# LucaHermes/ddrl

Hardware: AMD Instinct MI355X
Metric: env-steps/sec at 4096 envs × 4 leg agents; PPO update ms/minibatch (higher is better)
Workload: dtype fp32

## Files before the change

### ddrl_amd/csrc/common.h

```cpp
#pragma once
#include <hip/hip_runtime.h>
#include <stdint.h>

typedef float floatx4 __attribute__((ext_vector_type(4)));
typedef unsigned v4u __attribute__((ext_vector_type(4)));

#define DDRL_H 64
#ifndef DDRL_MB
#define DDRL_MB 128
#endif
#define DDRL_LOG2PI 1.8378770664093453

#ifndef DDRL_LDS_PAD
#define DDRL_LDS_PAD 1
#endif
constexpr bool kLdsPad = DDRL_LDS_PAD != 0;
__host__ __device__ constexpr int lds_rs(bool pad) { return pad ? 80 : 64; }
__host__ __device__ constexpr int lds_blk(bool pad) { return 16 * lds_rs(pad); }
__host__ __device__ constexpr int lds_img(int rows, bool pad) { return rows * lds_rs(pad); }
#define DDRL_LBLK lds_blk(kLdsPad)
#define DDRL_LIMG(rows) lds_img(rows, kLdsPad)
template <bool PAD = kLdsPad>
__device__ __forceinline__ int swz(int row) { return PAD ? (row & 0xB) : (((row >> 1) & 7) << 1); }
template <bool PAD = kLdsPad>
// ... 303 lines not shown
    }
}

template <int RT, bool PAD = kLdsPad>
__device__ __forceinline__ void layer2_bwd_rt(const NetLds& W, const floatx4 (*dz2)[4], floatx4 (*dh1)[4]) {
  constexpr int BLK = lds_blk(PAD);
#pragma unroll
  for (int t = 0; t < RT; ++t)
#pragma unroll
    for (int fb = 0; fb < 4; ++fb) dh1[t][fb] = splat4(0.f);
  const int wb[4] = {wbase<PAD>(0), wbase<PAD>(1), wbase<PAD>(2), wbase<PAD>(3)};
  auto ld = [&](int k, float* a) {
    const float* wp = W.w2 + wb[k & 3] + 16 * (k >> 2);
#pragma unroll
    for (int fb = 0; fb < 4; ++fb) a[fb] = wp[BLK * fb];
  };
  float wr[3][4];
  ld(0, wr[0]);
  ld(1, wr[1]);
#pragma unroll
  for (int k = 0; k < 16; ++k) {
    if (k + 2 < 16) ld(k + 2, wr[(k + 2) % 3]);
#pragma unroll
    for (int fb = 0; fb < 4; ++fb)
#pragma unroll
      for (int t = 0; t < RT; ++t) dh1[t][fb] = mfma4(wr[k % 3][fb], dz2[t][k >> 2][k & 3], dh1[t][fb]);
    __builtin_amdgcn_sched_barrier(0);
  }
}
__device__ __forceinline__ void layer2_bwd(const NetLds& W, const floatx4 dz2[4], floatx4 dh1[4]) {
  layer2_bwd_rt<1>(W, reinterpret_cast<const floatx4 (*)[4]>(dz2), reinterpret_cast<floatx4 (*)[4]>(dh1));
}

__device__ __forceinline__ void store_act(float* buf, int tile, const floatx4 v[4]) {
#pragma unroll
  for (int r = 0; r < 4; ++r) {
    float* p = buf + wbase(r) + DDRL_LBLK * tile;
#pragma unroll
    for (int fb = 0; fb < 4; ++fb) p[16 * fb] = v[fb][r];
  }
}

#define FM_LD 136
template <int LD = FM_LD>
__device__ __forceinline__ void store_act_fm(float* buf, int tile, const floatx4 v[4]) {
  const int lane = threadIdx.x & 63, c = lane & 15, q = lane >> 4;
  float* p = buf + (4 * q) * LD + 16 * tile + c;
#pragma unroll
  for (int fb = 0; fb < 4; ++fb)
#pragma unroll
    for (int r = 0; r < 4; ++r) p[(16 * fb + r) * LD] = v[fb][r];
}

template <int NROWS, int NT_, int LD = NROWS + 8, bool AHEAD = true>
__device__ __forceinline__ void dw_tiles_fm(const float* A, const float* B, const int* fa, int fo, floatx4* out) {
  const int lane = threadIdx.x & 63, c = lane & 15, q = lane >> 4;
#pragma unroll
  for (int i = 0; i < NT_; ++i) out[i] = splat4(0.f);
  const float* bp = B + (16 * fo + c) * LD + 4 * q;
  const float* ap[NT_];
#pragma unroll
  for (int i = 0; i < NT_; ++i) ap[i] = A + (16 * fa[i] + c) * LD + 4 * q;
  constexpr int NU = NROWS / 16;
  floatx4 bv[2], av[2][NT_];
  if constexpr (!AHEAD) {
    bv[0] = *reinterpret_cast<const floatx4*>(bp);
#pragma unroll
    for (int i = 0; i < NT_; ++i) av[0][i] = *reinterpret_cast<const floatx4*>(ap[i]);
#pragma unroll
    for (int u = 0; u < NU; ++u) {
      if (u + 1 < NU) {
        bv[(u + 1) & 1] = *reinterpret_cast<const floatx4*>(bp + 16 * (u + 1));
#pragma unroll
        for (int i = 0; i < NT_; ++i) av[(u + 1) & 1][i] = *reinterpret_cast<const floatx4*>(ap[i] + 16 * (u + 1));
      }
#pragma unroll
      for (int i = 0; i < NT_; ++i)
#pragma unroll
        for (int v = 0; v < 4; ++v) out[i] = mfma4(av[u & 1][i][v], bv[u & 1][v], out[i]);
      __builtin_amdgcn_sched_barrier(0);
    }
  } else {
    auto ld = [&](int u, int j) {
      if (j < NT_) av[u & 1][j] = *reinterpret_cast<const floatx4*>(ap[j] + 16 * u);
      else bv[u & 1] = *reinterpret_cast<const floatx4*>(bp + 16 * u);
    };
    constexpr int NL = NT_ + 1, PER = (NL + 2) / 3;
#pragma unroll
    for (int j = 0; j < NL; ++j) ld(0, j);
#pragma unroll
    for (int u = 0; u < NU; ++u) {
      __builtin_amdgcn_sched_barrier(0);
#pragma unroll
      for (int v = 0; v < 4; ++v) {
        if (u + 1 < NU && v < 3) {
#pragma unroll
          for (int j = v * PER; j < (v + 1) * PER && j < NL; ++j) ld(u + 1, j);
          __builtin_amdgcn_sched_barrier(0);
        }
#pragma unroll
        for (int i = 0; i < NT_; ++i) out[i] = mfma4(av[u & 1][i][v], bv[u & 1][v], out[i]);
        __builtin_amdgcn_sched_barrier(0);
      }
    }
  }
}

template <int NROWS>
__device__ __forceinline__ floatx4 dw_tile(const float* A, const float* B, int fa, int fo) {
  floatx4 acc = splat4(0.f);
  const int rb[4] = {rbase(0), rbase(1), rbase(2), rbase(3)};
  const float* ap = A + 16 * fa;
  const float* bp = B + 16 * fo;
#pragma unroll 2
  for (int u = 0; u < NROWS / 16; ++u) {
#pragma unroll
    for (int v = 0; v < 4; ++v) acc = mfma4(ap[rb[v] + DDRL_LBLK * u], bp[rb[v] + DDRL_LBLK * u], acc);
  }
  return acc;
}

template <int NROWS>
__device__ __forceinline__ void dw_tile2(const float* A, const float* B, int fa0, int fo0, int fa1, int fo1,
                                         floatx4& t0, floatx4& t1) {
  floatx4 a0 = splat4(0.f), a1 = splat4(0.f);
  const int rb[4] = {rbase(0), rbase(1), rbase(2), rbase(3)};
  const float *ap0 = A + 16 * fa0, *bp0 = B + 16 * fo0, *ap1 = A + 16 * fa1, *bp1 = B + 16 * fo1;
#pragma unroll 2
  for (int u = 0; u < NROWS / 16; ++u) {
#pragma unroll
    for (int v = 0; v < 4; ++v) {
      const int o = rb[v] + DDRL_LBLK * u;
      a0 = mfma4(ap0[o], bp0[o], a0);
      a1 = mfma4(ap1[o], bp1[o], a1);
    }
  }
  t0 = a0;
  t1 = a1;
}

template <int O, int NROWS>
__device__ __forceinline__ floatx4 dw_tile_head(const float* A, const float* D, int fa) {
  const int lane = threadIdx.x & 63, c = lane & 15, q = lane >> 4;
  floatx4 acc = splat4(0.f);
  const int rb[4] = {rbase(0), rbase(1), rbase(2), rbase(3)};
  const float* ap = A + 16 * fa;
  const bool cv = c < O;
  const float* dp = D + q * O + (cv ? c : 0);
#pragma unroll 2
  for (int u = 0; u < NROWS / 16; ++u) {
#pragma unroll
// ... 8 lines not shown
```

### ddrl_amd/csrc/ppo_ffn_impl.h

```cpp
#pragma once
#include <atomic>
#include "common.h"
#include "kernels.h"
#include "ffn.h"
#include "ppo_loss.h"

#ifndef DDRL_FFN_AT
#define DDRL_FFN_AT 0
#endif

#ifndef DDRL_FFN_KSP
#define DDRL_FFN_KSP 0
#endif
#ifndef DDRL_FFN_GROUP
#define DDRL_FFN_GROUP 0
#endif
#if DDRL_FFN_GROUP && (DDRL_FFN_KSP != 2 || DDRL_FFN_AT || DDRL_MB != 128 || defined(DDRL_XCHG_ATOMIC) || \
                       defined(DDRL_BOUNDS) || defined(DDRL_STAMPS))
#error "the group unit builds the production fused row-split kernel only (KSP = 2, 128 rows, default protocol)"
#endif
#if DDRL_MB == 256
#if DDRL_FFN_KSP != 2 || DDRL_FFN_AT == 2
#error "the DDRL_MB = 256 units build the fused row-split kernels only (DDRL_FFN_KSP = 2, no peer mode)"
#endif
#if DDRL_FFN_AT
#define DDRL_FFN_LAUNCH launch_update_ffn_mb256_atomic
#else
#define DDRL_FFN_LAUNCH launch_update_ffn_mb256
#endif
#elif DDRL_MB != 128
#error "DDRL_MB must be 128 or 256"
#elif DDRL_FFN_KSP == 1
#define DDRL_FFN_LAUNCH launch_update_ffn_k1
#elif DDRL_FFN_AT == 2
#define DDRL_FFN_LAUNCH launch_update_ffn_peer
#elif DDRL_FFN_AT
#define DDRL_FFN_LAUNCH launch_update_ffn_atomic
#else
#define DDRL_FFN_LAUNCH launch_update_ffn
#endif
#if DDRL_FFN_AT || defined(DDRL_XCHG_ATOMIC)
#define DDRL_XCHG_IS_ATOMIC 1
#else
#define DDRL_XCHG_IS_ATOMIC 0
#endif
#define DDRL_XCHG_LXSYS (DDRL_FFN_AT == 2)
#define DDRL_LX_ON (!DDRL_XCHG_IS_ATOMIC || DDRL_XCHG_LXSYS)
#ifndef DDRL_HEAD_PF
#define DDRL_HEAD_PF 4
#endif
constexpr int kHeadPfMaxO = (DDRL_FFN_KSP == 2 && !DDRL_FFN_AT) ? DDRL_HEAD_PF : 0;

namespace {

// ... 98 lines not shown
  for (int i = threadIdx.x; i < 64 * OB; i += blockDim.x) W.wo[i] = th[bo.wo + i];
  for (int i = threadIdx.x; i < OB; i += blockDim.x) W.bo[i] = th[bo.bo + i];
}
template <int OB, int NT, bool PAD>
__device__ __forceinline__ void stage_branch_batched(const float* __restrict__ th, int d, const BranchOff& bo,
                                                     float* lds, NetLds& W, int ncup) {
  static_assert((48 * 64) % NT == 0 && (64 * 64) % NT == 0, "staging split");
  constexpr int N1 = 48 * 64 / NT, N2 = 64 * 64 / NT, NS = (64 * OB + OB + 128 + NT - 1) / NT;
  W.w1 = lds; W.w2 = W.w1 + lds_img(48, PAD); W.b1 = W.w2 + lds_img(64, PAD); W.b2 = W.b1 + 64;
  W.wo = W.b2 + 64; W.bo = W.wo + 64 * OB; W.cup = W.bo + OB;
  const int t = threadIdx.x;
  float a1[N1], a2[N2], as[NS];
#pragma unroll
  for (int k = 0; k < N1; ++k) {
    const int i = t + NT * k;
    a1[k] = (i >> 6) < d ? th[bo.w1 + i] : 0.f;
  }
#pragma unroll
  for (int k = 0; k < N2; ++k) a2[k] = th[bo.w2 + t + NT * k];
#pragma unroll
  for (int k = 0; k < NS; ++k) {
    int e = t + NT * k;
    float x = 0.f;
    if (e < 64 * OB) x = th[bo.wo + e];
    else if ((e -= 64 * OB) < OB) x = th[bo.bo + e];
    else if ((e -= OB) < 64) x = th[bo.b1 + e];
    else if ((e -= 64) < 64) x = th[bo.b2 + e];
    as[k] = x;
  }
  float ac = t < ncup ? th[bo.cup + t] : 0.f;
#pragma unroll
  for (int k = 0; k < N1; ++k) {
    const int i = t + NT * k;
    W.w1[sidx<PAD>(i >> 6, i & 63)] = a1[k];
  }
#pragma unroll
  for (int k = 0; k < N2; ++k) {
    const int i = t + NT * k;
    W.w2[sidx<PAD>(i >> 6, i & 63)] = a2[k];
  }
#pragma unroll
  for (int k = 0; k < NS; ++k) {
    int e = t + NT * k;
    if (e < 64 * OB) W.wo[e] = as[k];
    else if ((e -= 64 * OB) < OB) W.bo[e] = as[k];
    else if ((e -= OB) < 64) W.b1[e] = as[k];
    else if ((e -= 64) < 64) W.b2[e] = as[k];
  }
  if (t < ncup) W.cup[t] = ac;
}
__host__ __device__ constexpr int branch_lds_floats(bool pad) { return lds_img(48, pad) + lds_img(64, pad) + 128 + 64 * 16 + 16; }
__host__ __device__ constexpr bool update_pad(int A, int ksp) { return kLdsPad && !(A == 8 && DDRL_MB / ksp >= 128); }
__host__ __device__ constexpr bool update_hmf(int ksp) { return ksp == 2 && DDRL_MB / ksp == 64; }

template <int OB>
__device__ __forceinline__ void small_param(int e, const BranchOff& bo, const NetLds& W, int& pidx, float*& lp) {
  if (e < 64 * OB) { pidx = bo.wo + e; lp = W.wo + e; return; }
  e -= 64 * OB;
  if (e < OB) { pidx = bo.bo + e; lp = W.bo + e; return; }
  e -= OB;
  if (e < 64) { pidx = bo.b1 + e; lp = W.b1 + e; return; }
  e -= 64;
  if (e < 64) { pidx = bo.b2 + e; lp = W.b2 + e; return; }
  e -= 64;
  pidx = bo.cup + e; lp = W.cup + e;
}


template <int A, int RT>
struct RowData {
  float x[RT][12];
  float act[RT][A];
  float ol[RT][2 * A];
  float s0[RT], s1[RT];
  int cid[RT];
};

template <int NW, int ROWS>
struct RowGather {
  static constexpr int MI = (ROWS * 20 + 64 * (NW - 1) - 1) / (64 * (NW - 1));
  const float* src[MI];
};
template <int NW, int ROWS>
__device__ __forceinline__ void rows_prepare(RowGather<NW, ROWS>& G, const float* rec, int stride, int cpr, int cpr_l,
                                             float inv_cpr_l, const int* idxb, int R) {
  constexpr int MI = RowGather<NW, ROWS>::MI;
  const int lane = threadIdx.x & 63, w = __builtin_amdgcn_readfirstlane(threadIdx.x >> 6);
#pragma unroll
  for (int it = 0; it < MI; ++it) G.src[it] = rec;
  if (w == NW - 1) return;
  const int nchunk = ROWS * cpr_l;
  int idx[MI], kk[MI];
#pragma unroll
  for (int it = 0; it < MI; ++it) {
    const int g = 64 * w + 64 * (NW - 1) * it + lane;
    int row = (int)(((float)g + 0.5f) * inv_cpr_l);
    kk[it] = min(g - row * cpr_l, cpr - 1);
    idx[it] = 0;
    if (g < nchunk) {
      if (!BCHK(row >= 0 && row < ROWS && kk[it] >= 0, 0)) row = 0;
      idx[it] = idxb[row];
    }
  }
#pragma unroll
  for (int it = 0; it < MI; ++it) {
    int i = idx[it];
// ... 316 lines not shown
  for (;;) {
#pragma unroll
    for (int j = 0; j < NQ; ++j)
      asm volatile("buffer_load_dwordx4 %0, %1, %2, %3 offen sc1" : "=v"(g[j]) : "v"(voff), "s"(rs), "s"(j * 4096));
    __builtin_amdgcn_sched_barrier(0);
    if (first) after_first();
    __builtin_amdgcn_sched_barrier(0);
    asm volatile("s_waitcnt vmcnt(0)" ::: "memory");
#pragma unroll
    for (int j = 0; j < NQ; ++j) asm volatile("" : "+v"(g[j]));
    unsigned bad = 0;
#pragma unroll
    for (int j = 0; j < NQ; ++j) bad |= (g[j][0] ^ bit) | (g[j][1] ^ bit) | (g[j][2] ^ bit) | (g[j][3] ^ bit);
#ifdef DDRL_STAMPS
    if (first && __builtin_amdgcn_ballot_w64((bad & 1u) != 0)) ++stale;
#endif
    first = false;
    if ((bad & 1u) == 0) break;
    if (xchg_abandon(t0, err)) {
#pragma unroll
      for (int j = 0; j < NQ; ++j) g[j] = v4u{0u, 0u, 0u, 0u};
      lost = true;
      break;
    }
    __builtin_amdgcn_s_sleep(1);
  }
  (void)stale;
#pragma unroll
  for (int j = 0; j < NQ; ++j)
#pragma unroll
    for (int k = 0; k < 4; ++k) out[4 * j + k] = __uint_as_float(g[j][k]);
  return lost;
}
#endif
#endif

template <int O>
__device__ __forceinline__ void head_bwd_mfma(const NetLds& W, const float* dout, floatx4 dh[4]) {
  static_assert(O % 4 == 0, "policy head: 2A outputs");
  const int lane = threadIdx.x & 63, c = lane & 15, q = lane >> 4;
  float b[O / 4];
#pragma unroll
  for (int kk = 0; kk < O / 4; ++kk)
    b[kk] = q == 0 ? dout[4 * kk] : q == 1 ? dout[4 * kk + 1] : q == 2 ? dout[4 * kk + 2] : dout[4 * kk + 3];
#pragma unroll
  for (int fb = 0; fb < 4; ++fb) {
    floatx4 acc = splat4(0.f);
#pragma unroll
    for (int kk = 0; kk < O / 4; ++kk) acc = mfma4(W.wo[(16 * fb + c) * O + 4 * kk + q], b[kk], acc);
    dh[fb] = acc;
  }
}

template <int NROWS, int NT_, int LD = NROWS + 8>
__device__ __forceinline__ void dw_tiles_fm_head(const float* A, const float* B, const int* fa, int fo, floatx4* out,
                                                 const float* AH, const float* BH, int fah, floatx4& outh) {
  const int lane = threadIdx.x & 63, c = lane & 15, q = lane >> 4;
#pragma unroll
  for (int i = 0; i < NT_; ++i) out[i] = splat4(0.f);
  outh = splat4(0.f);
  const float* bp = B + (16 * fo + c) * LD + 4 * q;
  const float* bph = BH + c * LD + 4 * q;
  const float* aph = AH + (16 * fah + c) * LD + 4 * q;
  const float* ap[NT_];
#pragma unroll
  for (int i = 0; i < NT_; ++i) ap[i] = A + (16 * fa[i] + c) * LD + 4 * q;
  constexpr int NU = NROWS / 16;
  floatx4 bv[2], av[2][NT_], bhv[2], ahv[2];
  auto ld = [&](int u, int j) {
    if (j < NT_) av[u & 1][j] = *reinterpret_cast<const floatx4*>(ap[j] + 16 * u);
    else if (j == NT_) bv[u & 1] = *reinterpret_cast<const floatx4*>(bp + 16 * u);
    else if (j == NT_ + 1) ahv[u & 1] = *reinterpret_cast<const floatx4*>(aph + 16 * u);
    else bhv[u & 1] = *reinterpret_cast<const floatx4*>(bph + 16 * u);
  };
  constexpr int NL = NT_ + 3, PER = (NL + 2) / 3;
#pragma unroll
  for (int j = 0; j < NL; ++j) ld(0, j);
#pragma unroll
  for (int u = 0; u < NU; ++u) {
    __builtin_amdgcn_sched_barrier(0);
#pragma unroll
    for (int v = 0; v < 4; ++v) {
      if (u + 1 < NU && v < 3) {
#pragma unroll
        for (int j = v * PER; j < (v + 1) * PER && j < NL; ++j) ld(u + 1, j);
        __builtin_amdgcn_sched_barrier(0);
      }
#pragma unroll
      for (int i = 0; i < NT_; ++i) out[i] = mfma4(av[u & 1][i][v], bv[u & 1][v], out[i]);
      outh = mfma4(ahv[u & 1][v], bhv[u & 1][v], outh);
      __builtin_amdgcn_sched_barrier(0);
    }
  }
}

template <int A, int KS1, int OB, bool POL, int NW, int KSP, bool CUP, bool LSBX>
__device__ __forceinline__ void update_loop(const UpdateArgs& U, const UpdateBatch& ub, float* lds, int p, int kq) {
  constexpr int ROWS = DDRL_MB / KSP;
  constexpr int NT = Geo<NW, ROWS>::NT, RT = Geo<NW, ROWS>::RT, NS1 = Geo<NW, ROWS>::NS1, NS2 = Geo<NW, ROWS>::NS2;
  constexpr bool PAD = update_pad(A, KSP);
  constexpr bool DWF = KSP != 1;
  const int wkq = ub.own_kq < 0 ? 0 : ub.own_kq;
  const UpdateHyper& H = ub.h;
  const int d = U.d;
  const FfnOffsets of = ffn_offsets(d, A);
  const BranchOff bo = branch_off(of, POL);
  const int nf1 = (d + 15) >> 4;
  constexpr int NSB0 = 64 * OB + OB + 128;
  constexpr int NCUP = CUP ? ncup_slots(OB, POL) : 0;
  constexpr int NSB = NSB0 + NCUP;
  constexpr bool cup = NCUP > 0;
  constexpr int nsb = NSB;
  constexpr int NSLOT = (NSB + NT - 1) / NT;
  constexpr int NSTAT = POL ? 3 : 5;
  constexpr int NTS = NS1 + NS2;
  constexpr int NP0 = (NSLOT + 2) / 2;
  constexpr int NP = NP0 + 2 * NTS;
  static_assert(KSP == 1 || (NT == 256 && NP == gx_pairs(OB, NW) && NP <= GX_MAX_PAIRS), "exchange pairs");
  constexpr bool LX = LSBX && KSP == 2 && DDRL_LX_ON;
  constexpr int NQ0 = (NSLOT + 1 + 3) / 4;
  constexpr int NQ = NQ0 + NTS;
  static_assert(!LX || NQ <= GX_MAX_PAIRS, "exchange quads");

  NetLds W;
  constexpr int LD = ROWS + 8;
  float* bufA = lds + branch_lds_floats(PAD);
  float* bufB = bufA + 64 * LD;
  float* Pb = bufB + 64 * LD;
  float* red = Pb + NW * NSB;
  int* idxb = reinterpret_cast<int*>(red + 128);
  static_assert(ROWS <= 128 && ROWS <= NT, "idxb holds 128 rows, one staging slot per thread");
  constexpr bool HMF = POL && update_hmf(KSP);
  float* bufH = red + 256;
  float* bufD = bufH + 64 * LD;
  float* stg = red + 256 + (HMF ? 80 * LD : 0);
  const int stride = U.lay.stride, cpr = stride >> 2, cpr_l = stg_chunks(stride, A);
  const float inv_cpr_l = 1.f / (float)cpr_l;

  const int tid = threadIdx.x, lane = tid & 63, c = lane & 15, q = lane >> 4,
            w = __builtin_amdgcn_readfirstlane(tid >> 6);
  constexpr bool coh = false;
  int row_l[RT];
  bool row_ok[RT];
#pragma unroll
  for (int t = 0; t < RT; ++t) {
    row_l[t] = 16 * RT * w + 16 * t + c;
    row_ok[t] = ROWS * kq + row_l[t] < ub.nrows;
  }

  const int total_steps = U.n_epochs * U.nb;
  const int last = U.max_steps >= 0 ? min(total_steps, U.step0 + U.max_steps) : total_steps;
  const int gr = ROWS * kq + tid;
  const bool gok = tid < ROWS && gr < ub.nrows;
  if (tid < ROWS) idxb[tid] = U.step0 < last && gok ? row_index(U, U.step0, gr, true) : 0;
  __syncthreads();
  if (U.step0 < last) issue_rows<NW, ROWS>(U.rec, stride, cpr, cpr_l, inv_cpr_l, idxb, stg, U.R, ub.lds_bytes);
  stage_branch_batched<OB, NT, PAD>(U.theta, d, bo, lds, W, NCUP);
  if constexpr (HMF) {
    for (int i = tid; i < NW * NSB; i += NT) Pb[i] = 0.f;
    for (int i = tid; i < 16 * LD; i += NT) bufD[i] = 0.f;
  }

  floatx4 mt[NTS], vt4[NTS];
  bool tv[NTS];
  int tfa[NTS], tfo[NTS];
#pragma unroll
  for (int i = 0; i < NTS; ++i) {
    const int tt = i < NS1 ? w + NW * i : w + NW * (i - NS1);
    tv[i] = i < NS1 ? true : (tt < 4 * nf1);
    tfa[i] = tt >> 2;
    tfo[i] = tt & 3;
#pragma unroll
    for (int r = 0; r < 4; ++r) {
      const int f = 16 * tfa[i] + 4 * q + r, o = 16 * tfo[i] + c;
      const bool ok = tv[i] && (i < NS1 || f < d) && !U.grad_out;
      const int pidx = (i < NS1 ? bo.w2 : bo.w1) + f * 64 + o;
      BCHK(!ok || (pidx >= 0 && pidx < of.n), 5);
      mt[i][r] = ok ? U.m[pidx] : 0.f;
      vt4[i][r] = ok ? U.v[pidx] : 0.f;

    }
  }
  float ms[NSLOT], vs[NSLOT];
  int sp_pidx[NSLOT], sp_lds[NSLOT];
#pragma unroll
  for (int k = 0; k < NSLOT; ++k) {
    const int e = tid + NT * k;
    ms[k] = vs[k] = 0.f;
    sp_pidx[k] = 0;
    sp_lds[k] = (int)(red + 127 - lds);
    if (e < nsb) {
      int pidx; float* lp;
      small_param<OB>(e, bo, W, pidx, lp);
      BCHK(pidx >= 0 && pidx < of.n + NCUP, 5);
      sp_pidx[k] = pidx;
      sp_lds[k] = (int)(lp - lds);
      if (!U.grad_out) {
        ms[k] = U.m[pidx];
        vs[k] = U.v[pidx];
      }
    }
  }
  int ebase[4];
#pragma unroll
  for (int r = 0; r < 4; ++r) ebase[r] = sidx<PAD>(4 * q + r, 16 * (w & 3) + c);
  float b1p = U.beta_pow[0], b2p = U.beta_pow[1];
  const float adv_mean = U.adv_norm[0], adv_den = U.adv_norm[1];
  const float beta = U.kl_coeff;
  const float lo = 1.f - H.clip, hi = 1.f + H.clip;
  __syncthreads();

  RowData<A, RT> cur;
  const unsigned xlast_bits = (KS1 < 12 && 4 * (KS1 - 1) + q >= d) ? 0u : 0xffffffffu;
  wait_vmcnt0();
  __syncthreads();
  if (tid < ROWS) idxb[tid] = U.step0 + 1 < last && gok ? row_index(U, U.step0 + 1, gr, true) : 0;
  int nxt = U.step0 + 2 < last && gok ? row_index(U, U.step0 + 2, gr, true) : 0;
  const size_t gx_branch = ((size_t)p * 2 + (POL ? 0 : 1)) * KSP;
  __syncthreads();

  const float inv_rows = 1.f / (float)ub.nrows;
  unsigned st_stale = 0;
  (void)st_stale;
  STAMP_INIT
  for (int step = U.step0; step < last; ++step) {
    const float alpha = H.lr * sqrtf(1.f - b2p) / (1.f - b1p);
    load_row<A, KS1, POL, RT>(stg, 4 * cpr_l, U.lay, row_l, d, cur, xlast_bits);
    floatx4 h1[RT][4], h2[RT][4], dz[RT][4];
    float out[RT][OB], dout[RT][OB];
    fwd_mark(-1);
    if constexpr (KSP == 2 && RT == 1 && OB <= kHeadPfMaxO && !(CUP && POL))
      ffn_fwd_rt<OB, KS1, RT, PAD, decltype(fwd_mark), true>(W, cur.x, h1, h2, out, fwd_mark);
    else ffn_fwd_rt<OB, KS1, RT, PAD>(W, cur.x, h1, h2, out, fwd_mark);
    float pre[RT][A], cf[RT][A];
    if constexpr (cup) {
      {
#pragma unroll
        for (int t = 0; t < RT; ++t)
#pragma unroll
          for (int j = 0; j < A; ++j) {
            pre[t][j] = out[t][j];
            cf[t][j] = W.cup[cur.cid[t] * A + j];
            out[t][j] *= cf[t][j];
          }
      }
    }
    fwd_mark(3);
    STAMP(0);
    float st[NSTAT];
#pragma unroll
    for (int k = 0; k < NSTAT; ++k) st[k] = 0.f;
#pragma unroll
    for (int t = 0; t < RT; ++t) {
      float st0[NSTAT];
      if constexpr (POL)
        policy_loss_row<A>(out[t], cur.act[t], cur.ol[t], cur.s0[t], (cur.s1[t] - adv_mean) / adv_den,
                           beta, lo, hi, H.ent_coeff, ub.inv_n, row_ok[t], dout[t], st0);
      else
        value_loss_row(out[t][0], cur.s0[t], cur.s1[t], H, ub.inv_n, row_ok[t], dout[t], st0);
#pragma unroll
      for (int k = 0; k < NSTAT; ++k) st[k] += st0[k];
    }
    STAMP(1);
    float* Pw = Pb + w * NSB;
    if constexpr (cup) {
      {
#pragma unroll
        for (int lg = 0; lg < 4; ++lg)
#pragma unroll
          for (int j = 0; j < A; ++j) {
            float v = 0.f;
#pragma unroll
            for (int t = 0; t < RT; ++t) v += cur.cid[t] == lg ? dout[t][j] * pre[t][j] : 0.f;
            v = row16_sum(v);
            if (lane == 0) Pw[NSB0 + lg * A + j] = v;
          }
#pragma unroll
        for (int t = 0; t < RT; ++t)
#pragma unroll
          for (int j = 0; j < A; ++j) dout[t][j] *= cf[t][j];
// ... 29 lines not shown
      float dsum = dout[0][o];
#pragma unroll
      for (int t = 1; t < RT; ++t) dsum += dout[t][o];
      const float s = row16_sum(dsum);
      if (lane == 0) Pw[64 * OB + o] = s;
    }
#pragma unroll
    for (int k = 0; k < NSTAT; ++k) {
      const float s = row16_sum(st[k]);
      if (lane == 0) red[w * 8 + k] = s;
    }
    STAMP(2);
#pragma unroll
    for (int t = 0; t < RT; ++t) {
      if constexpr (POL) head_bwd_mfma<OB>(W, dout[t], dz[t]);
      else head_bwd<OB>(W, dout[t], dz[t]);
      dtanh_inplace(dz[t], h2[t]);
    }
    {
      float v[16];
#pragma unroll
      for (int fb = 0; fb < 4; ++fb)
#pragma unroll
        for (int r = 0; r < 4; ++r) {
          v[4 * fb + r] = dz[0][fb][r];
#pragma unroll
          for (int t = 1; t < RT; ++t) v[4 * fb + r] += dz[t][fb][r];
        }
      Pw[64 * OB + OB + 64 + h_own] = row16_transpose_sum(v);
    }
#pragma unroll
    for (int t = 0; t < RT; ++t) {
      store_act_fm<LD>(bufA, RT * w + t, h1[t]);
      store_act_fm<LD>(bufB, RT * w + t, dz[t]);
    }
    STAMP(3);
#ifndef DDRL_ABL_NO_L2BWD
    layer2_bwd_rt<RT, PAD>(W, dz, h2);
#endif
#pragma unroll
    for (int t = 0; t < RT; ++t) dtanh_inplace(h2[t], h1[t]);
    {
      float v[16];
#pragma unroll
      for (int fb = 0; fb < 4; ++fb)
#pragma unroll
        for (int r = 0; r < 4; ++r) {
          v[4 * fb + r] = h2[0][fb][r];
#pragma unroll
          for (int t = 1; t < RT; ++t) v[4 * fb + r] += h2[t][fb][r];
        }
      Pw[64 * OB + OB + h_own] = row16_transpose_sum(v);
    }
    STAMP(4);
    __syncthreads();
    STAMP(5);
    const unsigned gtag = xchg_tag(ub.epoch, step);
    const int gstep = step + (int)ub.lx_base;
    const unsigned lbit = lx_bit(gstep);
    (void)lbit;
    const size_t gx_box = (size_t)GX_MAX_PAIRS * 256 * 2;
    const gx_box_t gx_mine = gx_rsrc(ub.gx + ((gx_branch + kq) * 2 + (gstep & 1)) * gx_box);
    float gs[NSLOT];
    float st_own = 0.f;
    auto put_small = [&] {
      float v0[2 * NP0];
#pragma unroll
      for (int k = 0; k < 2 * NP0; ++k) v0[k] = 0.f;
#pragma unroll
      for (int k = 0; k < NSLOT; ++k) {
        const int e = tid + NT * k;
        float sm = 0.f;
        if (e < nsb)
          for (int i = 0; i < NW; ++i) sm += Pb[i * NSB + e];
        gs[k] = sm;
        v0[k] = sm;
      }
      if (tid < NSTAT)
        for (int i = 0; i < NW; ++i) st_own += red[i * 8 + tid];
      v0[NSLOT] = st_own;
#if DDRL_LX_ON
      if constexpr (LX) {
        const lx_box_t lx_mine = lx_rsrc(ub.gx + ((gx_branch + kq) * 2 + (gstep & 1)) * gx_box);
        float w0[4 * NQ0];
#pragma unroll
        for (int k = 0; k < 4 * NQ0; ++k) w0[k] = k <= NSLOT ? v0[k] : 0.f;
#pragma unroll
        for (int j = 0; j < NQ0; ++j) gx_put4(lx_mine, j, w0[4 * j], w0[4 * j + 1], w0[4 * j + 2], w0[4 * j + 3], lbit);
        return;
      }
#endif
#pragma unroll
      for (int j = 0; j < NP0; ++j) gx_put(gx_mine, j, v0[2 * j], v0[2 * j + 1], gtag, coh);
    };
    if constexpr (KSP == 2 && !HMF) put_small();
    floatx4 gt[NTS];
    RowGather<NW, ROWS> G;
    (void)G;
#ifndef DDRL_ABL_NO_DW2
    if constexpr (HMF) {
      static_assert(NW == 4, "one head tile (16 features) per wave");
      static_assert(DWF, "the head tile's helper has the loads-ahead form only");
      floatx4 gh;
      dw_tiles_fm_head<ROWS, NS1, ROWS + 8>(bufA, bufB, tfa, w & 3, gt, bufH, bufD, w, gh);
      if (c < OB)
#pragma unroll
        for (int r = 0; r < 4; ++r) Pb[(16 * w + 4 * q + r) * OB + c] = gh[r];
    } else {
      dw_tiles_fm<ROWS, NS1, ROWS + 8, DWF>(bufA, bufB, tfa, w & 3, gt);
    }
#else
    for (int i = 0; i < NS1; ++i) gt[i] = splat4(0.f);
#endif
    if constexpr (KSP == 2) {
#pragma unroll
      for (int i = 0; i < NS1; ++i) {
#if DDRL_LX_ON
        if constexpr (LX) {
          gx_put4(lx_rsrc(ub.gx + ((gx_branch + kq) * 2 + (gstep & 1)) * gx_box), NQ0 + i, gt[i][0], gt[i][1], gt[i][2],
                  gt[i][3], lbit);
          continue;
        }
#endif
        gx_put(gx_mine, NP0 + 2 * i, gt[i][0], gt[i][1], gtag, coh);
        gx_put(gx_mine, NP0 + 2 * i + 1, gt[i][2], gt[i][3], gtag, coh);
      }
    }
    STAMP(6);
    __syncthreads();
    if constexpr (HMF) put_small();
    STAMP(7);
#pragma unroll
    for (int t = 0; t < RT; ++t) {
      store_act_fm<LD>(bufB, RT * w + t, h2[t]);
#pragma unroll
      for (int s = 0; s < 12; ++s) bufA[(4 * s + q) * LD + row_l[t]] = cur.x[t][s];
    }
    __syncthreads();
    STAMP(8);
#ifndef DDRL_ABL_NO_PREFETCH
    if (KSP == 1 && step + 1 < last) issue_rows<NW, ROWS>(U.rec, stride, cpr, cpr_l, inv_cpr_l, idxb, stg, U.R, ub.lds_bytes);
#endif
    const int xlane = 64 * (NW - 1);
    unsigned long long* const xmine = ub.xchg + (((size_t)p * 2 + (POL ? 0 : 1)) * KSP + kq) * 2 + (step & 1);
    unsigned long long* const xother = ub.xchg + (((size_t)p * 2 + (POL ? 1 : 0)) * KSP + kq) * 2 + (step & 1);
    unsigned long long xv = 0;
    if (tid == xlane) xv = xchg_load(xother);
    STAMP(9);
    {
#pragma unroll
      for (int i = NS1; i < NTS; ++i) gt[i] = splat4(0.f);
      int n1 = 0;
#pragma unroll
      for (int i = NS1; i < NTS; ++i) n1 += tv[i] ? 1 : 0;
#ifdef DDRL_ABL_NO_DW1
      n1 = -1;
#endif
      if (n1 == NS2) dw_tiles_fm<ROWS, NS2, ROWS + 8, DWF>(bufA, bufB, tfa + NS1, w & 3, gt + NS1);
      else if constexpr (NS2 >= 3) {
        if (n1 == 2) dw_tiles_fm<ROWS, 2, ROWS + 8, DWF>(bufA, bufB, tfa + NS1, w & 3, gt + NS1);
        else if (n1 == 1) dw_tiles_fm<ROWS, 1, ROWS + 8, DWF>(bufA, bufB, tfa + NS1, w & 3, gt + NS1);
      } else if (n1 == 1) dw_tiles_fm<ROWS, 1, ROWS + 8, DWF>(bufA, bufB, tfa + NS1, w & 3, gt + NS1);
    }
    STAMP(10);
    if constexpr (KSP == 2) {
#pragma unroll
      for (int i = NS1; i < NTS; ++i) {
#if DDRL_LX_ON
        if constexpr (LX) {
          gx_put4(lx_rsrc(ub.gx + ((gx_branch + kq) * 2 + (gstep & 1)) * gx_box), NQ0 + i, gt[i][0], gt[i][1], gt[i][2],
                  gt[i][3], lbit);
          continue;
        }
#endif
        gx_put(gx_mine, NP0 + 2 * i, gt[i][0], gt[i][1], gtag, coh);
        gx_put(gx_mine, NP0 + 2 * i + 1, gt[i][2], gt[i][3], gtag, coh);
      }
#if DDRL_LX_ON
      if constexpr (LX) {
        float o4[4 * NQ];
#ifdef DDRL_LX_ASMPOLL
        asm volatile("" : "+v"(xv));
        gx_get4c<NQ>(ub.gx + ((gx_branch + (kq ^ 1)) * 2 + (gstep & 1)) * gx_box, lbit, o4, ub.err, st_stale, [&] {
          rows_prepare<NW, ROWS>(G, U.rec, stride, cpr, cpr_l, inv_cpr_l, idxb, U.R);
        });
#else
        gx_get4<NQ>(lx_rsrc(ub.gx + ((gx_branch + (kq ^ 1)) * 2 + (gstep & 1)) * gx_box), lbit, o4, ub.err, [&] {
          if (step + 1 < last) issue_rows<NW, ROWS>(U.rec, stride, cpr, cpr_l, inv_cpr_l, idxb, stg, U.R, ub.lds_bytes);
        });
#endif
#pragma unroll
        for (int k = 0; k < NSLOT; ++k) gs[k] = lx_t(gs[k], lbit) + o4[k];
        if (tid < NSTAT) red[96 + tid] = lx_t(st_own, lbit) + o4[NSLOT];
#pragma unroll
        for (int i = 0; i < NTS; ++i)
#pragma unroll
          for (int r = 0; r < 4; ++r) gt[i][r] = lx_t(gt[i][r], lbit) + o4[4 * (NQ0 + i) + r];
      } else
#endif
      {
      float o[2 * NP];
#ifndef DDRL_ABL_NO_PREFETCH
      gx_get<NP>(gx_rsrc(ub.gx + ((gx_branch + (kq ^ 1)) * 2 + (gstep & 1)) * gx_box), gtag, o, ub.err, [&] {
        if (step + 1 < last) issue_rows<NW, ROWS>(U.rec, stride, cpr, cpr_l, inv_cpr_l, idxb, stg, U.R, ub.lds_bytes);
      });
#else
      gx_get<NP>(gx_rsrc(ub.gx + ((gx_branch + (kq ^ 1)) * 2 + (gstep & 1)) * gx_box), gtag, o, ub.err, [] {});
#endif
      if constexpr (LSBX) {
#pragma unroll
        for (int k = 0; k < NSLOT; ++k) gs[k] = lx_t(gs[k], lbit) + lx_t(o[k], lbit);
        if (tid < NSTAT) red[96 + tid] = lx_t(st_own, lbit) + lx_t(o[NSLOT], lbit);
#pragma unroll
        for (int i = 0; i < NTS; ++i)
#pragma unroll
// ... 180 lines not shown
  }
}

#if DDRL_FFN_GROUP
struct GroupBatch {
  const UpdateArgs* table;
  int n_chains;
  UpdateBatch b;
};
template <int A, int KS1, bool CUP>
__global__ void __launch_bounds__(64 * waves_for(A, 2)) k_update_ffn_group(GroupBatch gb) {
  extern __shared__ float lds[];
  constexpr int NW = waves_for(A, 2);
  const int c = 8 * (int)(blockIdx.x >> 5) + (int)(blockIdx.x & 7);
  if (threadIdx.x == 0) {
    unsigned x;
    asm volatile("s_getreg_b32 %0, hwreg(HW_REG_XCC_ID)" : "=s"(x));
    gb.b.xcc[blockIdx.x] = (int)(x & 0xf);
  }
  if (c >= gb.n_chains) return;
  const int j = (int)(blockIdx.x >> 3) & 3, branch = j >> 1, kq = j & 1;
  constexpr int NWORD = (int)(sizeof(UpdateArgs) / sizeof(unsigned));
  static_assert(sizeof(UpdateArgs) % sizeof(unsigned) == 0, "UpdateArgs in whole words");
  const unsigned* src = reinterpret_cast<const unsigned*>(gb.table + c);
  unsigned wd[NWORD];
#pragma unroll
  for (int k = 0; k < NWORD; ++k) wd[k] = (unsigned)__builtin_amdgcn_readfirstlane((int)src[k]);
  UpdateArgs U;
  __builtin_memcpy(&U, wd, sizeof(U));
  if (branch) update_loop<A, KS1, 1, false, NW, 2, false, true>(U, gb.b, lds, c, kq);
  else update_loop<A, KS1, 2 * A, true, NW, 2, CUP, true>(U, gb.b, lds, c, kq);
}
#else
template <int A, int KS1, int KSP, bool CUP, bool LSBX>
__global__ void __launch_bounds__(64 * waves_for(A, KSP)) k_update_ffn(UpdateBatch ub) {
  extern __shared__ float lds[];
  constexpr int NW = waves_for(A, KSP);
  const int p = blockIdx.x & 7;
  if (threadIdx.x == 0) {
    unsigned x;
    asm volatile("s_getreg_b32 %0, hwreg(HW_REG_XCC_ID)" : "=s"(x));
    ub.xcc[blockIdx.x] = (int)(x & 0xf);
  }
  if (p >= ub.h.P) return;
  const int j = blockIdx.x >> 3, branch = j / KSP, kq = j - branch * KSP;
  if (ub.own_kq >= 0 && kq != ub.own_kq) return;
  const UpdateArgs U = ub.a[p];
  if (branch) update_loop<A, KS1, 1, false, NW, KSP, false, LSBX>(U, ub, lds, p, kq);
  else update_loop<A, KS1, 2 * A, true, NW, KSP, CUP, LSBX>(U, ub, lds, p, kq);
}

#endif

static size_t update_lds_bytes(int O, int stride, int ksp) {
  const int nsb = 64 * O + O + 128 + ncup_slots(O, true);
  const int nw = waves_for(O / 2, ksp);
  return (size_t)(branch_lds_floats(update_pad(O / 2, ksp)) + 2 * 64 * (DDRL_MB / ksp + 8) + nw * nsb + 256 +
                  (update_hmf(ksp) ? 80 * (DDRL_MB / ksp + 8) : 0) +
                  (DDRL_MB / ksp) * 4 * stg_chunks(stride, O / 2)) * 4;
}

#if DDRL_FFN_GROUP
template <int A, int KS1, bool CUP = false>
static void launch_group_t(hipStream_t s, GroupBatch& gb, int stride, int grid) {
  gb.b.lds_bytes = (unsigned)update_lds_bytes(2 * A, stride, 2);
  hipLaunchKernelGGL((k_update_ffn_group<A, KS1, CUP>), dim3(grid), dim3(64 * waves_for(A, 2)), gb.b.lds_bytes, s, gb);
}

}

int update_group_grid(int n_chains) { return 32 * ((n_chains - 1) >> 3) + 24 + ((n_chains - 1) & 7) + 1; }

int launch_update_ffn_group(hipStream_t s, const UpdateArgs* table_dev, int n_chains, const UpdateHyper& h, int A, int d,
                            int stride, int cup, unsigned long long* xchg, unsigned long long* gx, int* err,
                            unsigned* epoch_ctr, int* xcc) {
  if (n_chains < 1) return -1;
  GroupBatch gb;
  gb.table = table_dev;
  gb.n_chains = n_chains;
  gb.b.h = h;
  gb.b.nrows = DDRL_MB;
  gb.b.inv_n = 1.f / DDRL_MB;
  gb.b.xchg = xchg;
  gb.b.gx = gx;
  gb.b.err = err;
  gb.b.xcc = xcc;
  gb.b.own_kq = -1;
  gb.b.lx_base = 0;
  gb.b.epoch = (*epoch_ctr)++ % 4095u + 1u;
  const int rows8 = 8 * ((n_chains + 7) >> 3);
  if (gb.b.epoch == 1) (void)hipMemsetAsync(xchg, 0, sizeof(unsigned long long) * 8 * (size_t)rows8, s);
  (void)hipMemsetAsync(gx, 0, gx_bytes(n_chains), s);
  const int grid = update_group_grid(n_chains);
  if (cup)
    launch_group_t<2, 5, true>(s, gb, stride, grid);
  else
    DDRL_DISPATCH_A_KS1(A, d, launch_group_t, s, gb, stride, grid);
  return 0;
}
#else
template <int A, int KS1, bool CUP = false>
static void launch_update_t(hipStream_t s, UpdateBatch& ub, int P, int stride, int ksp, bool lx) {
  ub.lds_bytes = (unsigned)update_lds_bytes(2 * A, stride, ksp);
#if DDRL_FFN_KSP != 1
  if (ksp == 2 && lx)
    hipLaunchKernelGGL((k_update_ffn<A, KS1, 2, CUP, true>), dim3(24 + P), dim3(64 * waves_for(A, 2)), ub.lds_bytes, s, ub);
#endif
#if DDRL_FFN_KSP != 2
  if (ksp == 2 && !lx)
    hipLaunchKernelGGL((k_update_ffn<A, KS1, 2, CUP, false>), dim3(24 + P), dim3(64 * waves_for(A, 2)), ub.lds_bytes, s, ub);
  if (ksp == 1)
    hipLaunchKernelGGL((k_update_ffn<A, KS1, 1, CUP, false>), dim3(8 + P), dim3(64 * waves_for(A, 1)), ub.lds_bytes, s, ub);
#endif
}

}

void DDRL_FFN_LAUNCH(hipStream_t s, const UpdateArgs* ua, const UpdateHyper& h, int nrows, float inv_n,
                       int A, int d, int stride, int cup, unsigned long long* xchg, unsigned long long* gx, int ksp,
                       int* err, unsigned* epoch_ctr, int* xcc, int own_kq, unsigned lx_base) {
#if DDRL_MB == 256
  if (!(ksp == 2 && ua[0].grad_out == nullptr && own_kq < 0 && nrows == DDRL_MB)) {
    (void)hipMemsetD32Async((hipDeviceptr_t)err, 1, 1, s);
    return;
  }
#elif DDRL_FFN_KSP == 2
  if (!(ksp == 2 && ua[0].grad_out == nullptr)) {
    launch_update_ffn_k1(s, ua, h, nrows, inv_n, A, d, stride, cup, xchg, gx, ksp, err, epoch_ctr, xcc, own_kq, lx_base);
    return;
  }
#endif
  UpdateBatch ub;
  for (int p = 0; p < DDRL_MAXP; ++p) ub.a[p] = p < h.P ? ua[p] : UpdateArgs{};
  ub.h = h;
  ub.nrows = nrows;
  ub.inv_n = inv_n;
  ub.xchg = xchg;
  ub.gx = gx;
  ub.err = err;
  ub.xcc = xcc;
  ub.own_kq = own_kq;
  ub.lx_base = lx_base;
  ub.epoch = (*epoch_ctr)++ % 4095u + 1u;
  const bool lx = ksp == 2 && ua[0].grad_out == nullptr;
  if (ub.epoch == 1) (void)hipMemsetAsync(xchg, 0, sizeof(unsigned long long) * 8 * DDRL_MAXP, s);
  if (own_kq < 0 && (ub.epoch == 1 || (lx && DDRL_LX_ON))) {
    const int s0 = ua[0].step0;
    const unsigned b0 = (((unsigned)s0 >> 1) & 1u) ^ 1u, b1 = (((unsigned)(s0 + 1) >> 1) & 1u) ^ 1u;
    if (!(lx && DDRL_LX_ON) || (b0 && b1)) {
      (void)hipMemsetAsync(gx, 0, gx_bytes(DDRL_MAXP), s);
    } else {
      const size_t box = sizeof(unsigned long long) * (size_t)GX_MAX_PAIRS * 256 * 2;
      const size_t nbox = gx_bytes(DDRL_MAXP) / box;
      for (int q = 0; q < 2; ++q) {
        const unsigned first_bit = (s0 & 1) == q ? b0 : b1;
// ... 11 lines not shown
```

Measured before the change: 1.291 million.

## Stage X and dZ1 images in dedicated LDS to drop a barrier and chain dW loads

Adds dedicated LDS buffers for the input X and the layer-1 activation/gradient image. They are written early in the step, so the layer-1 weight-gradient tiles no longer need bufA/bufB to be rewritten behind an extra __syncthreads. The first dW tile loop now prefetches the operands of the next tile group into registers during its last iteration, and the small-parameter reduction is split into phases so it can run before the barrier. This removes one or two block-wide barriers and an LDS rewrite per step, at the cost of more LDS per block (checked against 160 KB) and more register pressure.

```diff
diff --git a/ddrl_amd/csrc/common.h b/ddrl_amd/csrc/common.h
--- a/ddrl_amd/csrc/common.h
+++ b/ddrl_amd/csrc/common.h
@@ -379,8 +379,12 @@
     for (int r = 0; r < 4; ++r) p[(16 * fb + r) * LD] = v[fb][r];
 }
 
-template <int NROWS, int NT_, int LD = NROWS + 8, bool AHEAD = true>
-__device__ __forceinline__ void dw_tiles_fm(const float* A, const float* B, const int* fa, int fo, floatx4* out) {
+template <int NROWS, int NT_, int LD = NROWS + 8, bool AHEAD = true, bool PRE = false, int NN = 0>
+__device__ __forceinline__ void dw_tiles_fm(const float* A, const float* B, const int* fa, int fo, floatx4* out,
+                                            const floatx4* pav = nullptr, const floatx4* pbv = nullptr,
+                                            const float* NA = nullptr, const float* NB = nullptr,
+                                            const int* nfa = nullptr, floatx4* nav = nullptr, floatx4* nbv = nullptr) {
+  static_assert(AHEAD || (!PRE && NN == 0), "chained streams have the loads-ahead form only");
   const int lane = threadIdx.x & 63, c = lane & 15, q = lane >> 4;
 #pragma unroll
   for (int i = 0; i < NT_; ++i) out[i] = splat4(0.f);
@@ -412,9 +416,20 @@
       if (j < NT_) av[u & 1][j] = *reinterpret_cast<const floatx4*>(ap[j] + 16 * u);
       else bv[u & 1] = *reinterpret_cast<const floatx4*>(bp + 16 * u);
     };
+    auto nld = [&](int j) {
+      if (j < NN) nav[j] = *reinterpret_cast<const floatx4*>(NA + (16 * nfa[j] + c) * LD + 4 * q);
+      else *nbv = *reinterpret_cast<const floatx4*>(NB + (16 * fo + c) * LD + 4 * q);
+    };
     constexpr int NL = NT_ + 1, PER = (NL + 2) / 3;
-#pragma unroll
-    for (int j = 0; j < NL; ++j) ld(0, j);
+    constexpr int NNL = NN + 1, NPER = (NNL + 2) / 3;
+    if constexpr (PRE) {
+#pragma unroll
+      for (int j = 0; j < NT_; ++j) av[0][j] = pav[j];
+      bv[0] = *pbv;
+    } else {
+#pragma unroll
+      for (int j = 0; j < NL; ++j) ld(0, j);
+    }
 #pragma unroll
     for (int u = 0; u < NU; ++u) {
       __builtin_amdgcn_sched_barrier(0);
@@ -424,6 +439,13 @@
 #pragma unroll
           for (int j = v * PER; j < (v + 1) * PER && j < NL; ++j) ld(u + 1, j);
           __builtin_amdgcn_sched_barrier(0);
+        }
+        if constexpr (NN > 0) {
+          if (u + 1 == NU && v < 3) {
+#pragma unroll
+            for (int j = v * NPER; j < (v + 1) * NPER && j < NNL; ++j) nld(j);
+            __builtin_amdgcn_sched_barrier(0);
+          }
         }
 #pragma unroll
         for (int i = 0; i < NT_; ++i) out[i] = mfma4(av[u & 1][i][v], bv[u & 1][v], out[i]);
diff --git a/ddrl_amd/csrc/ppo_ffn_impl.h b/ddrl_amd/csrc/ppo_ffn_impl.h
--- a/ddrl_amd/csrc/ppo_ffn_impl.h
+++ b/ddrl_amd/csrc/ppo_ffn_impl.h
@@ -1,5 +1,6 @@
 #pragma once
 #include <atomic>
+#include <type_traits>
 #include "common.h"
 #include "kernels.h"
 #include "ffn.h"
@@ -204,6 +205,13 @@
 __host__ __device__ constexpr int branch_lds_floats(bool pad) { return lds_img(48, pad) + lds_img(64, pad) + 128 + 64 * 16 + 16; }
 __host__ __device__ constexpr bool update_pad(int A, int ksp) { return kLdsPad && !(A == 8 && DDRL_MB / ksp >= 128); }
 __host__ __device__ constexpr bool update_hmf(int ksp) { return ksp == 2 && DDRL_MB / ksp == 64; }
+#ifndef DDRL_DWB_MAXA
+#define DDRL_DWB_MAXA 4
+#endif
+static_assert(DDRL_DWB_MAXA <= 4, "the A = 8 kernels have no LDS for the X / dZ1 images");
+__host__ __device__ constexpr bool update_dwb(int A, int ksp) {
+  return !DDRL_FFN_AT && DDRL_FFN_KSP != 1 && ksp == 2 && DDRL_MB / ksp == 64 && A <= DDRL_DWB_MAXA;
+}
 
 template <int OB>
 __device__ __forceinline__ void small_param(int e, const BranchOff& bo, const NetLds& W, int& pidx, float*& lp) {
@@ -626,9 +634,12 @@
   }
 }
 
-template <int NROWS, int NT_, int LD = NROWS + 8>
+template <int NROWS, int NT_, int LD = NROWS + 8, int NN = 0>
 __device__ __forceinline__ void dw_tiles_fm_head(const float* A, const float* B, const int* fa, int fo, floatx4* out,
-                                                 const float* AH, const float* BH, int fah, floatx4& outh) {
+                                                 const float* AH, const float* BH, int fah, floatx4& outh,
+                                                 const float* NA = nullptr, const float* NB = nullptr,
+                                                 const int* nfa = nullptr, floatx4* nav = nullptr,
+                                                 floatx4* nbv = nullptr) {
   const int lane = threadIdx.x & 63, c = lane & 15, q = lane >> 4;
 #pragma unroll
   for (int i = 0; i < NT_; ++i) out[i] = splat4(0.f);
@@ -647,7 +658,12 @@
     else if (j == NT_ + 1) ahv[u & 1] = *reinterpret_cast<const floatx4*>(aph + 16 * u);
     else bhv[u & 1] = *reinterpret_cast<const floatx4*>(bph + 16 * u);
   };
+  auto nld = [&](int j) {
+    if (j < NN) nav[j] = *reinterpret_cast<const floatx4*>(NA + (16 * nfa[j] + c) * LD + 4 * q);
+    else *nbv = *reinterpret_cast<const floatx4*>(NB + (16 * fo + c) * LD + 4 * q);
+  };
   constexpr int NL = NT_ + 3, PER = (NL + 2) / 3;
+  constexpr int NNL = NN + 1, NPER = (NNL + 2) / 3;
 #pragma unroll
   for (int j = 0; j < NL; ++j) ld(0, j);
 #pragma unroll
@@ -659,6 +675,13 @@
 #pragma unroll
         for (int j = v * PER; j < (v + 1) * PER && j < NL; ++j) ld(u + 1, j);
         __builtin_amdgcn_sched_barrier(0);
+      }
+      if constexpr (NN > 0) {
+        if (u + 1 == NU && v < 3) {
+#pragma unroll
+          for (int j = v * NPER; j < (v + 1) * NPER && j < NNL; ++j) nld(j);
+          __builtin_amdgcn_sched_barrier(0);
+        }
       }
 #pragma unroll
       for (int i = 0; i < NT_; ++i) out[i] = mfma4(av[u & 1][i][v], bv[u & 1][v], out[i]);
@@ -707,7 +730,13 @@
   constexpr bool HMF = POL && update_hmf(KSP);
   float* bufH = red + 256;
   float* bufD = bufH + 64 * LD;
-  float* stg = red + 256 + (HMF ? 80 * LD : 0);
+  constexpr bool DWB = update_dwb(A, KSP);
+  constexpr bool SMB = DWB && HMF && 64 * OB == NT;
+  constexpr bool KEEP2 = DWB && HMF && !SMB;
+  constexpr bool DWPRE = DWB && !KEEP2 && DWF;
+  float* bufX = red + 256 + (HMF ? 80 * LD : 0);
+  float* bufZ1 = bufX + 48 * LD;
+  float* stg = red + 256 + (HMF ? 80 * LD : 0) + (DWB ? 112 * LD : 0);
   const int stride = U.lay.stride, cpr = stride >> 2, cpr_l = stg_chunks(stride, A);
   const float inv_cpr_l = 1.f / (float)cpr_l;
 
@@ -800,6 +829,12 @@
   for (int step = U.step0; step < last; ++step) {
     const float alpha = H.lr * sqrtf(1.f - b2p) / (1.f - b1p);
     load_row<A, KS1, POL, RT>(stg, 4 * cpr_l, U.lay, row_l, d, cur, xlast_bits);
+    if constexpr (DWB) {
+#pragma unroll
+      for (int t = 0; t < RT; ++t)
+#pragma unroll
+        for (int s = 0; s < 12; ++s) bufX[(4 * s + q) * LD + row_l[t]] = cur.x[t][s];
+    }
     floatx4 h1[RT][4], h2[RT][4], dz[RT][4];
     float out[RT][OB], dout[RT][OB];
     fwd_mark(-1);
@@ -935,6 +970,9 @@
         }
       Pw[64 * OB + OB + h_own] = row16_transpose_sum(v);
     }
+    if constexpr (DWB)
+#pragma unroll
+      for (int t = 0; t < RT; ++t) store_act_fm<LD>(bufZ1, RT * w + t, h2[t]);
     STAMP(4);
     __syncthreads();
     STAMP(5);
@@ -946,12 +984,19 @@
     const gx_box_t gx_mine = gx_rsrc(ub.gx + ((gx_branch + kq) * 2 + (gstep & 1)) * gx_box);
     float gs[NSLOT];
     float st_own = 0.f;
-    auto put_small = [&] {
+    auto put_small_ph = [&](auto phase) {
+      constexpr int PH = decltype(phase)::value;
       float v0[2 * NP0];
 #pragma unroll
       for (int k = 0; k < 2 * NP0; ++k) v0[k] = 0.f;
 #pragma unroll
       for (int k = 0; k < NSLOT; ++k) {
+        if constexpr (PH != 0) {
+          if (PH == 2 || k == 0) {
+            v0[k] = gs[k];
+            continue;
+          }
+        }
         const int e = tid + NT * k;
         float sm = 0.f;
         if (e < nsb)
@@ -959,8 +1004,11 @@
         gs[k] = sm;
         v0[k] = sm;
       }
-      if (tid < NSTAT)
-        for (int i = 0; i < NW; ++i) st_own += red[i * 8 + tid];
+      if constexpr (PH != 2) {
+        if (tid < NSTAT)
+          for (int i = 0; i < NW; ++i) st_own += red[i * 8 + tid];
+      }
+      if constexpr (PH == 1) return;
       v0[NSLOT] = st_own;
 #if DDRL_LX_ON
       if constexpr (LX) {
@@ -976,24 +1024,40 @@
 #pragma unroll
       for (int j = 0; j < NP0; ++j) gx_put(gx_mine, j, v0[2 * j], v0[2 * j + 1], gtag, coh);
     };
+    auto put_small = [&] { put_small_ph(std::integral_constant<int, 0>()); };
     if constexpr (KSP == 2 && !HMF) put_small();
+    if constexpr (SMB) put_small_ph(std::integral_constant<int, 1>());
     floatx4 gt[NTS];
     RowGather<NW, ROWS> G;
     (void)G;
+    floatx4 pav[NS2], pbv;
+    (void)pav; (void)pbv;
 #ifndef DDRL_ABL_NO_DW2
     if constexpr (HMF) {
       static_assert(NW == 4, "one head tile (16 features) per wave");
       static_assert(DWF, "the head tile's helper has the loads-ahead form only");
       floatx4 gh;
-      dw_tiles_fm_head<ROWS, NS1, ROWS + 8>(bufA, bufB, tfa, w & 3, gt, bufH, bufD, w, gh);
+      if constexpr (DWPRE)
+        dw_tiles_fm_head<ROWS, NS1, ROWS + 8, NS2>(bufA, bufB, tfa, w & 3, gt, bufH, bufD, w, gh, bufX, bufZ1, tfa + NS1,
+                                                   pav, &pbv);
+      else
+        dw_tiles_fm_head<ROWS, NS1, ROWS + 8>(bufA, bufB, tfa, w & 3, gt, bufH, bufD, w, gh);
       if (c < OB)
 #pragma unroll
         for (int r = 0; r < 4; ++r) Pb[(16 * w + 4 * q + r) * OB + c] = gh[r];
     } else {
-      dw_tiles_fm<ROWS, NS1, ROWS + 8, DWF>(bufA, bufB, tfa, w & 3, gt);
+      if constexpr (DWPRE)
+        dw_tiles_fm<ROWS, NS1, ROWS + 8, DWF, false, NS2>(bufA, bufB, tfa, w & 3, gt, nullptr, nullptr, bufX, bufZ1,
+                                                          tfa + NS1, pav, &pbv);
+      else
+        dw_tiles_fm<ROWS, NS1, ROWS + 8, DWF>(bufA, bufB, tfa, w & 3, gt);
     }
 #else
     for (int i = 0; i < NS1; ++i) gt[i] = splat4(0.f);
+    if constexpr (DWPRE) {
+      for (int i = 0; i < NS2; ++i) pav[i] = *reinterpret_cast<const floatx4*>(bufX + (16 * tfa[NS1 + i] + c) * LD + 4 * q);
+      pbv = *reinterpret_cast<const floatx4*>(bufZ1 + (16 * (w & 3) + c) * LD + 4 * q);
+    }
 #endif
     if constexpr (KSP == 2) {
 #pragma unroll
@@ -1009,17 +1073,24 @@
         gx_put(gx_mine, NP0 + 2 * i + 1, gt[i][2], gt[i][3], gtag, coh);
       }
     }
+    if constexpr (SMB) {
+      __builtin_amdgcn_wave_barrier();
+      gs[0] = 0.f + Pb[tid];
+      put_small_ph(std::integral_constant<int, 2>());
+    }
     STAMP(6);
-    __syncthreads();
-    if constexpr (HMF) put_small();
+    if constexpr (!DWB || KEEP2) __syncthreads();
+    if constexpr (HMF && !SMB) put_small();
     STAMP(7);
-#pragma unroll
-    for (int t = 0; t < RT; ++t) {
-      store_act_fm<LD>(bufB, RT * w + t, h2[t]);
-#pragma unroll
-      for (int s = 0; s < 12; ++s) bufA[(4 * s + q) * LD + row_l[t]] = cur.x[t][s];
-    }
-    __syncthreads();
+    if constexpr (!DWB) {
+#pragma unroll
+      for (int t = 0; t < RT; ++t) {
+        store_act_fm<LD>(bufB, RT * w + t, h2[t]);
+#pragma unroll
+        for (int s = 0; s < 12; ++s) bufA[(4 * s + q) * LD + row_l[t]] = cur.x[t][s];
+      }
+      __syncthreads();
+    }
     STAMP(8);
 #ifndef DDRL_ABL_NO_PREFETCH
     if (KSP == 1 && step + 1 < last) issue_rows<NW, ROWS>(U.rec, stride, cpr, cpr_l, inv_cpr_l, idxb, stg, U.R, ub.lds_bytes);
@@ -1039,11 +1110,23 @@
 #ifdef DDRL_ABL_NO_DW1
       n1 = -1;
 #endif
-      if (n1 == NS2) dw_tiles_fm<ROWS, NS2, ROWS + 8, DWF>(bufA, bufB, tfa + NS1, w & 3, gt + NS1);
-      else if constexpr (NS2 >= 3) {
-        if (n1 == 2) dw_tiles_fm<ROWS, 2, ROWS + 8, DWF>(bufA, bufB, tfa + NS1, w & 3, gt + NS1);
-        else if (n1 == 1) dw_tiles_fm<ROWS, 1, ROWS + 8, DWF>(bufA, bufB, tfa + NS1, w & 3, gt + NS1);
-      } else if (n1 == 1) dw_tiles_fm<ROWS, 1, ROWS + 8, DWF>(bufA, bufB, tfa + NS1, w & 3, gt + NS1);
+      if constexpr (!DWB) {
+        if (n1 == NS2) dw_tiles_fm<ROWS, NS2, ROWS + 8, DWF>(bufA, bufB, tfa + NS1, w & 3, gt + NS1);
+        else if constexpr (NS2 >= 3) {
+          if (n1 == 2) dw_tiles_fm<ROWS, 2, ROWS + 8, DWF>(bufA, bufB, tfa + NS1, w & 3, gt + NS1);
+          else if (n1 == 1) dw_tiles_fm<ROWS, 1, ROWS + 8, DWF>(bufA, bufB, tfa + NS1, w & 3, gt + NS1);
+        } else if (n1 == 1) dw_tiles_fm<ROWS, 1, ROWS + 8, DWF>(bufA, bufB, tfa + NS1, w & 3, gt + NS1);
+      } else {
+        auto dw1 = [&](auto nt) {
+          constexpr int N1 = decltype(nt)::value;
+          dw_tiles_fm<ROWS, N1, ROWS + 8, DWF, DWPRE>(bufX, bufZ1, tfa + NS1, w & 3, gt + NS1, pav, &pbv);
+        };
+        if (n1 == NS2) dw1(std::integral_constant<int, NS2>());
+        else if constexpr (NS2 >= 3) {
+          if (n1 == 2) dw1(std::integral_constant<int, 2>());
+          else if (n1 == 1) dw1(std::integral_constant<int, 1>());
+        } else if (n1 == 1) dw1(std::integral_constant<int, 1>());
+      }
     }
     STAMP(10);
     if constexpr (KSP == 2) {
@@ -1330,17 +1413,23 @@
 
 #endif
 
-static size_t update_lds_bytes(int O, int stride, int ksp) {
+static constexpr size_t update_lds_bytes(int O, int stride, int ksp) {
   const int nsb = 64 * O + O + 128 + ncup_slots(O, true);
   const int nw = waves_for(O / 2, ksp);
   return (size_t)(branch_lds_floats(update_pad(O / 2, ksp)) + 2 * 64 * (DDRL_MB / ksp + 8) + nw * nsb + 256 +
                   (update_hmf(ksp) ? 80 * (DDRL_MB / ksp + 8) : 0) +
+                  (update_dwb(O / 2, ksp) ? (48 + 64) * (DDRL_MB / ksp + 8) : 0) +
                   (DDRL_MB / ksp) * 4 * stg_chunks(stride, O / 2)) * 4;
+}
+template <int A, int KS1, bool CUP>
+constexpr bool update_lds_fits() {
+  return !update_dwb(A, 2) || update_lds_bytes(2 * A, (4 * KS1 + 3 * A + 5 + (CUP ? 1 : 0) + 3) & ~3, 2) <= 160 * 1024;
 }
 
 #if DDRL_FFN_GROUP
 template <int A, int KS1, bool CUP = false>
 static void launch_group_t(hipStream_t s, GroupBatch& gb, int stride, int grid) {
+  static_assert(update_lds_fits<A, KS1, CUP>(), "X / dZ1 images: past the 160 KB of LDS at the widest record");
   gb.b.lds_bytes = (unsigned)update_lds_bytes(2 * A, stride, 2);
   hipLaunchKernelGGL((k_update_ffn_group<A, KS1, CUP>), dim3(grid), dim3(64 * waves_for(A, 2)), gb.b.lds_bytes, s, gb);
 }
@@ -1379,6 +1468,7 @@
 #else
 template <int A, int KS1, bool CUP = false>
 static void launch_update_t(hipStream_t s, UpdateBatch& ub, int P, int stride, int ksp, bool lx) {
+  static_assert(update_lds_fits<A, KS1, CUP>(), "X / dZ1 images: past the 160 KB of LDS at the widest record");
   ub.lds_bytes = (unsigned)update_lds_bytes(2 * A, stride, ksp);
 #if DDRL_FFN_KSP != 1
   if (ksp == 2 && lx)
```

Measured after the change: 1.305 million (median of 6 runs). 1.1% higher.
